# linto-ai/ssak

Hardware: AMD Instinct MI355X
Metric: utterances/sec (16 kHz, 10 s) Wav2Vec2-base CTC train step (higher is better)
Workload: dtype bf16; 1 GPU; Wav2Vec2-base CTC fine-tune step, bf16, synthetic 10 s @16 kHz utterances (BASELINE.json configs[1]; DP over xGMI for n_gpus>1 = configs[2]); per_gpu_batch=32, global_batch=32, samples_per_utt=160000, frames=499, frozen_feature_encoder=True, regularisers=script defaults (dropout/layerdrop/specaugment on), parallelism=dp1

## Files before the change

include/ssak_hip.h:

```cpp
#ifndef SSAK_HIP_H
#define SSAK_HIP_H
#include <stddef.h>
#include <stdint.h>

#ifdef __cplusplus
extern "C" {
#endif

#define SSAK_OK 0
#define SSAK_ERR_INVALID (-1)
#define SSAK_ERR_LAUNCH (-2)
#define SSAK_ERR_STATE (-3)

#define SSAK_REDUCTION_SUM 0
#define SSAK_REDUCTION_MEAN 1

int ssak_version(void);
const char* ssak_last_error(void);

size_t ssak_wave_normalize_workspace_bytes(int B, int T);
int ssak_wave_normalize(const float* in, const int32_t* lens, int B, int T, float* out, int32_t* mask,
                        void* workspace, size_t workspace_bytes, void* stream);

size_t ssak_logmel_table_floats(void);
// ... 344 lines not shown
int ssak_test_attn_adapter_fwd(const void* y, const void* res, const float* ln_g, const float* ln_b, const void* w1, const float* b1,
                               const void* w2, const float* b2, const float* next_g, const float* next_b, void* r_out, void* out,
                               float* mean, float* rstd, int M, int H, int A, float eps_adapter, float eps_next, int dtype,
                               void* stream);

int ssak_debug_posconv_prepare(const float* g, const float* v, void* wf, void* wb, float* norms, int H, int G, int K, int dtype,
                               void* stream);
int ssak_debug_posconv_pack(const void* h, void* pg, int B, int F, int H, int G, int K, int dtype, void* stream);
size_t ssak_debug_posconv_workspace_bytes(int B, int F, int H, int G, int K);
int ssak_debug_posconv_direct(const void* h, const void* w, const float* bias, void* out, void* pre, int B, int F, int H, int G, int K,
                              int row0, int gelu, void* workspace, size_t workspace_bytes, void* stream);
int ssak_debug_posconv_wgrad(const void* h, const void* dpre, float* dwf, int B, int F, int H, int G, int K, void* workspace,
                             size_t workspace_bytes, void* stream);
int ssak_debug_posconv_weight_bwd(const float* dwf, const float* g, const float* v, float* norms, float* dg, float* dv, int H, int G,
                                  int K, void* stream);

size_t ssak_debug_conv0_bwd_workspace_bytes(int B, int T, int C);
int ssak_debug_conv0_bwd(const float* x, const float* w, const float* gamma, const float* beta, const void* dy, const double* sums,
                         float* dw, float* dgamma, float* dbeta, int B, int T, int C, int dtype, void* workspace, size_t workspace_bytes,
                         void* stream);
size_t ssak_debug_conv0_wgrad_workspace_bytes(int B, int C, int ksize);
int ssak_debug_conv0_wgrad(const void* d, const float* x, float* dw, int B, int T, int C, int ksize, int stride, int dtype, void* workspace,
                           size_t workspace_bytes, void* stream);
int ssak_debug_conv0_bias(const float* x, const float* w, const float* bias, void* out, int B, int T, int C, int dtype, void* stream);
int ssak_debug_col2im(const void* dxcol, void* dx, int B, int Tin, int Tout, int C, int k, int s, int dtype, void* stream);
int ssak_debug_sum_slabs(const float* slabs, int nb, long n, float* out, void* stream);
int ssak_debug_conv_weight_rearrange(const float* w, void* out, int Co, int Ci, int k, int dtype, void* stream);
int ssak_debug_conv_wgrad_unrearrange(const float* dwr, float* g, int Co, int Ci, int k, void* stream);
int ssak_debug_col2im_k3s2(const void* dxcol, const void* pre, void* out, int B, int F, int Tin, int RS1, int H, int dtype, void* stream);
int ssak_debug_mel_to_cl(const float* mel, void* cl, int B, int C, int T, int RS, int lead, int dtype, void* stream);
// ... 8 lines not shown
```

ssak_amd/csrc/api.cpp:

```cpp
#include <stdarg.h>
#include <stdio.h>

#include <string.h>

#include <mutex>
#include <vector>

#include "kernels.h"

static thread_local char g_err[512] = "";

void ssak_set_error(const char* fmt, ...) {
  va_list ap;
  va_start(ap, fmt);
  vsnprintf(g_err, sizeof(g_err), fmt, ap);
  va_end(ap);
}

extern "C" int ssak_version(void) { return 630; }
extern "C" const char* ssak_last_error(void) { return g_err; }

#include <atomic>
#include <map>
namespace {
struct ProfRec {
  hipEvent_t e0, e1;
  int slot;
  double work;
};
struct ProfStream {
  int mode = 0;
  std::vector<char> want;
  std::vector<ProfRec> recs;
};
// ... 155 lines not shown
```

ssak_amd/csrc/kernels.h:

```cpp
#pragma once
#include "common.h"

enum : int {
  PROF_ATTN_FWD = 0, PROF_ATTN_BWD, PROF_LN_FWD, PROF_LN_BWD, PROF_CONV0, PROF_ADAMW, PROF_SUMSQ, PROF_CTC, PROF_WAVE_NORM,
  PROF_ROWWISE, PROF_POSCONV_W, PROF_SOFTMAX, PROF_POSCONV_DIRECT, PROF_POSCONV_WGRAD, PROF_LOGMEL,
  PROF_CLASS_SLOTS
};
constexpr int PROF_MAX_SLOTS = 128;
int ssak_prof_register(const char* name, int bound);
bool ssak_prof_wanted(int slot, hipStream_t st);
class ProfScope {
 public:
  ProfScope(int slot, double work, hipStream_t st);
  ~ProfScope();
  ProfScope(const ProfScope&) = delete;
  ProfScope& operator=(const ProfScope&) = delete;

 private:
  hipStream_t st_;
  hipEvent_t e0_ = nullptr;
  int slot_;
  double work_;
  bool on_;
};
// ... 49 lines not shown
                    hipStream_t st);
template <typename T>
int k_colsum_t(const T* X, long ld, int M, int N, float* out, hipStream_t st, float* scratch = nullptr, size_t scratch_floats = 0,
               const uint8_t* rowmask = nullptr, const int32_t* flens = nullptr, int F = 0);
int k_cast_f32_bf16(const float* in, bf16* out, long n, hipStream_t st);
template <typename T>
int k_specaug_fwd_t(T* h, const uint8_t* mask, const int32_t* flens, const float* embed, int B, int F, int C,
                    hipStream_t st);
template <typename T>
int k_specaug_bwd_t(T* dh, const uint8_t* mask, const int32_t* flens, float* dembed, int B, int F, int C,
                    hipStream_t st, float* scratch = nullptr, size_t scratch_floats = 0);
template <typename T>
int k_gelu_grad_mul_t(const T* dy, const T* pre, T* out, long n, hipStream_t st);
template <typename T>
int k_add_t(const T* a, const T* b, T* out, long n, hipStream_t st);
int k_layernorm_fwd(const bf16* y, const bf16* res, const float* gamma, const float* beta, bf16* r_out, bf16* out,
                    float* mean, float* rstd, int M, int C, float eps, const DropSpec& pre, const DropSpec& post,
                    hipStream_t st, const DropSpec& mid = DropSpec(), bool post_gelu = false);
int k_layernorm_bwd(const bf16* g1, const bf16* g2, const bf16* r, const float* mean, const float* rstd,
                    const float* gamma, const bf16* g_res, bf16* dr, bf16* dy, float* dgamma, float* dbeta,
                    float* partial, int M, int C, const DropSpec& pre, const DropSpec& post,
                    hipStream_t st, const DropSpec& mid = DropSpec(), float* dy_colsum = nullptr,
                    const float* post_gelu_beta = nullptr);
int k_colsum(const bf16* X, long ld, int M, int N, float* out, hipStream_t st, float* scratch = nullptr, size_t scratch_floats = 0,
             const uint8_t* rowmask = nullptr, const int32_t* flens = nullptr, int F = 0);

size_t k_conv0_stats_doubles(int B, int T0, int C);
template <typename T>
int k_conv0_gn_gelu_t(const float* x, const float* w, const float* gamma, const float* beta, T* out, double* stats,
                      int B, int Tn, int T0, int C, int ksize, int stride, hipStream_t st, bool raw_input = false);
// ... 77 lines not shown
```

ssak_amd/csrc/norm_act.hip:

```cpp
#include <algorithm>
#include <type_traits>

#include "common.h"
#include "kernels.h"

namespace {

SSAK_DEFINE_DROP_TABLE

constexpr int ROW_THREADS = 256;
template <int VEC>
__device__ __forceinline__ void load_colmul(uint32_t (&cm)[VEC], int col0) {
#pragma unroll
  for (int k = 0; k < VEC; k += 4) {
    const uint4 t = *reinterpret_cast<const uint4*>(g_drop_colmul.v + col0 + k);
    cm[k] = t.x, cm[k + 1] = t.y, cm[k + 2] = t.z, cm[k + 3] = t.w;
  }
}

template <typename T, int VEC>
using ChunkT = typename std::conditional<VEC == 8, Chunk8<T>, Chunk4<T>>::type;
template <typename T, int VEC>
__device__ __forceinline__ ChunkT<T, VEC> f_to_chunk(const float* f) {
  if constexpr (VEC == 8) return f_to_chunk8<T>(f);
// ... 604 lines not shown
}
__global__ __launch_bounds__(1024) void colsum_rows_kernel(const float* __restrict__ partial, int slots, int N, float* __restrict__ out) {
  __shared__ float red[16][65];
  const int cx = threadIdx.x & 63, ry = threadIdx.x >> 6;
  const int n = blockIdx.x * 64 + cx;
  float s = 0.f;
  if (n < N)
    for (int k = ry; k < slots; k += 16) s += partial[(long)k * N + n];
  red[ry][cx] = s;
  __syncthreads();
  if (ry == 0 && n < N) {
    float t = 0.f;
#pragma unroll
    for (int r = 0; r < 16; ++r) t += red[r][cx];
    out[n] += t;
  }
}

__global__ void cast_f32_bf16_kernel(const float* __restrict__ in, bf16* __restrict__ out, long n) {
  const long i = ((long)blockIdx.x * blockDim.x + threadIdx.x) * 4;
  if (i + 3 < n) {
    const float4 q = *reinterpret_cast<const float4*>(in + i);
    const bf16x4 t = {(bf16)q.x, (bf16)q.y, (bf16)q.z, (bf16)q.w};
    *reinterpret_cast<bf16x4*>(out + i) = t;
  } else {
    for (long j = i; j < n; ++j) out[j] = (bf16)in[j];
  }
}

template <typename T>
// ... 208 lines not shown
               const uint8_t* rowmask, const int32_t* flens, int F) {
  SSAK_REQUIRE(M > 0 && N > 0 && (N & 7) == 0 && (ld & 7) == 0, "colsum: N=%d ld=%ld must be multiples of 8", N, ld);
  dim3 grid(ssak_cdiv(N, 64), min(64, ssak_cdiv(M, 32)));
  ProfScope prof_scope(PROF_ROWWISE, (double)M * N * sizeof(T), st);
  const bool det = scratch && scratch_floats >= (size_t)grid.y * N;
  colsum_kernel<T><<<grid, 256, 0, st>>>(X, ld, M, N, out, det ? scratch : nullptr, rowmask, flens, F > 0 ? F : 1);
  SSAK_LAUNCH_CHECK();
  if (det) {
    if (g_reduce_sink && g_reduce_sink->push(scratch, N, (int)grid.y, N, out)) return SSAK_OK;
    colsum_rows_kernel<<<ssak_cdiv(N, 64), 1024, 0, st>>>(scratch, (int)grid.y, N, out);
    SSAK_LAUNCH_CHECK();
  }
  return SSAK_OK;
}

thread_local ReduceSink* g_reduce_sink = nullptr;

int k_colsum_rows(const float* partial, int slots, int N, float* out, hipStream_t st) {
  ProfScope prof_scope(PROF_ROWWISE, (double)slots * N * 4.0, st);
  colsum_rows_kernel<<<ssak_cdiv(N, 64), 1024, 0, st>>>(partial, slots, N, out);
  SSAK_LAUNCH_CHECK();
  return SSAK_OK;
}

int k_reduce_flush(ReduceSink& sink, hipStream_t st) {
  int done = 0;
  double bytes = 0.0;
  for (int i = 0; i < sink.n; ++i) bytes += (double)sink.jobs[i].slots * sink.jobs[i].ncols * 4.0;
  ProfScope prof_scope(PROF_ROWWISE, bytes, st);
  while (done < sink.n) {
// ... 64 lines not shown
  return SSAK_OK;
}

#define SSAK_INSTANTIATE_ROW_KERNELS(T)                                                                                           \
  template int k_layernorm_fwd_t<T>(const T*, const T*, const float*, const float*, T*, T*, float*, float*, int, int, float,      \
                                    const DropSpec&, const DropSpec&, hipStream_t, const DropSpec&, bool);                        \
  template int k_layernorm_bwd_t<T>(const T*, const T*, const T*, const float*, const float*, const float*, const T*, T*, T*,     \
                                    float*, float*, float*, int, int, const DropSpec&, const DropSpec&, hipStream_t,              \
                                    const DropSpec&, float*, const float*);                                                       \
  template int k_softmax_fwd_t<T>(const T*, T*, T*, const int32_t*, int, int, int, int, const DropSpec&, hipStream_t);            \
  template int k_softmax_bwd_t<T>(const T*, const T*, T*, int, int, int, const DropSpec&, hipStream_t);                           \
  template int k_colsum_t<T>(const T*, long, int, int, float*, hipStream_t, float*, size_t, const uint8_t*, const int32_t*, int); \
  template int k_specaug_fwd_t<T>(T*, const uint8_t*, const int32_t*, const float*, int, int, int, hipStream_t);                  \
  template int k_specaug_bwd_t<T>(T*, const uint8_t*, const int32_t*, float*, int, int, int, hipStream_t, float*, size_t);        \
  template int k_gelu_grad_mul_t<T>(const T*, const T*, T*, long, hipStream_t);                                                   \
  template int k_add_t<T>(const T*, const T*, T*, long, hipStream_t);
SSAK_INSTANTIATE_ROW_KERNELS(bf16)
SSAK_INSTANTIATE_ROW_KERNELS(float)

int k_layernorm_fwd(const bf16* y, const bf16* res, const float* gamma, const float* beta, bf16* r_out, bf16* out,
                    float* mean, float* rstd, int M, int C, float eps, const DropSpec& pre, const DropSpec& post,
                    hipStream_t st, const DropSpec& mid, bool post_gelu) {
  return k_layernorm_fwd_t<bf16>(y, res, gamma, beta, r_out, out, mean, rstd, M, C, eps, pre, post, st, mid, post_gelu);
}
int k_layernorm_bwd(const bf16* g1, const bf16* g2, const bf16* r, const float* mean, const float* rstd,
                    const float* gamma, const bf16* g_res, bf16* dr, bf16* dy, float* dgamma, float* dbeta,
                    float* partial, int M, int C, const DropSpec& pre, const DropSpec& post, hipStream_t st,
                    const DropSpec& mid, float* dy_colsum, const float* post_gelu_beta) {
  return k_layernorm_bwd_t<bf16>(g1, g2, r, mean, rstd, gamma, g_res, dr, dy, dgamma, dbeta, partial, M, C, pre, post, st, mid,
                                 dy_colsum, post_gelu_beta);
}
// ... 134 lines not shown
  SSAK_REQUIRE(debug_p_ok(p), "debug_softmax_bwd: p outside [0, 1)");
  const DropSpec d = debug_site(seed, site, p);
  if (dtype == 0) return k_softmax_bwd_t<bf16>((const bf16*)dPd, (const bf16*)P, (bf16*)dS, rows, cols, ld, d, (hipStream_t)stream);
  return k_softmax_bwd_t<float>((const float*)dPd, (const float*)P, (float*)dS, rows, cols, ld, d, (hipStream_t)stream);
}

extern "C" int ssak_debug_gelu(const float* x, long n, float* y, float* dydx, int dtype, void* stream) {
  SSAK_REQUIRE(dtype == 0 || dtype == 1, "debug_gelu: dtype %d (0 bf16, 1 fp32)", dtype);
  SSAK_REQUIRE(x && n > 0 && (y || dydx), "debug_gelu: bad arguments");
  const unsigned grid = (unsigned)((n + 255) / 256);
  if (dtype == 0) debug_gelu_kernel<bf16><<<grid, 256, 0, (hipStream_t)stream>>>(x, n, y, dydx);
  else debug_gelu_kernel<float><<<grid, 256, 0, (hipStream_t)stream>>>(x, n, y, dydx);
  SSAK_LAUNCH_CHECK();
  return SSAK_OK;
}
```

ssak_amd/csrc/optim.hip:

```cpp
#include "kernels.h"

namespace {

__global__ __launch_bounds__(256) void sumsq_kernel(const float* __restrict__ g, long n, float* __restrict__ out) {
  __shared__ float red[16];
  float s = 0.f;
  const long n4 = n >> 2;
  for (long i = (long)blockIdx.x * blockDim.x + threadIdx.x; i < n4; i += (long)gridDim.x * blockDim.x) {
    const float4 q = reinterpret_cast<const float4*>(g)[i];
    s += q.x * q.x + q.y * q.y + q.z * q.z + q.w * q.w;
  }
  if (blockIdx.x == 0)
    for (long i = (n4 << 2) + threadIdx.x; i < n; i += blockDim.x) s += g[i] * g[i];
  s = block_sum(s, red);
  if (threadIdx.x == 0) out[blockIdx.x] = s;
}
__global__ __launch_bounds__(1024) void sumsq_final_kernel(const float* __restrict__ partial, int n, float* __restrict__ out,
                                                           int add) {
  __shared__ float red[16];
  float s = threadIdx.x < n ? partial[threadIdx.x] : 0.f;
  s = block_sum(s, red);
  if (threadIdx.x == 0) out[0] = add ? out[0] + s : s;
}

__global__ __launch_bounds__(256) void adamw_kernel(float* __restrict__ p, const float* __restrict__ g,
                                                    float* __restrict__ m, float* __restrict__ v,
                                                    bf16* __restrict__ shadow, long n, const float* __restrict__ gnorm_sq,
                                                    float max_norm, float grad_scale, float lr, float beta1, float beta2,
                                                    float eps, float wd, float bc1, float bc2_sqrt) {
  float coef = grad_scale;
  if (gnorm_sq && max_norm > 0.f) {
    const float nrm = sqrtf(gnorm_sq[0]) * grad_scale;
    coef *= fminf(1.f, max_norm / (nrm + 1e-6f));
  }
  const float step_size = lr / bc1;
  const float decay = 1.f - lr * wd;
  const long n4 = n >> 2;
  for (long i = (long)blockIdx.x * blockDim.x + threadIdx.x; i < n4; i += (long)gridDim.x * blockDim.x) {
    float4 pp = reinterpret_cast<float4*>(p)[i];
    const float4 gg = reinterpret_cast<const float4*>(g)[i];
    float4 mm = reinterpret_cast<float4*>(m)[i];
    float4 vv = reinterpret_cast<float4*>(v)[i];
    float* pe = &pp.x;
    const float* ge = &gg.x;
    float* me = &mm.x;
    float* ve = &vv.x;
#pragma unroll
    for (int k = 0; k < 4; ++k) {
      const float gk = ge[k] * coef;
      me[k] = beta1 * me[k] + (1.f - beta1) * gk;
      ve[k] = beta2 * ve[k] + (1.f - beta2) * gk * gk;
      const float denom = sqrtf(ve[k]) / bc2_sqrt + eps;
      pe[k] = pe[k] * decay - step_size * (me[k] / denom);
    }
    reinterpret_cast<float4*>(p)[i] = pp;
    reinterpret_cast<float4*>(m)[i] = mm;
    reinterpret_cast<float4*>(v)[i] = vv;
    if (shadow) {
      const bf16x4 t = {(bf16)pp.x, (bf16)pp.y, (bf16)pp.z, (bf16)pp.w};
      reinterpret_cast<bf16x4*>(shadow)[i] = t;
    }
  }
  if (blockIdx.x == 0) {
    for (long i = (n4 << 2) + threadIdx.x; i < n; i += blockDim.x) {
      const float gk = g[i] * coef;
      const float mk = beta1 * m[i] + (1.f - beta1) * gk;
      const float vk = beta2 * v[i] + (1.f - beta2) * gk * gk;
      m[i] = mk;
      v[i] = vk;
      const float pk = p[i] * decay - step_size * (mk / (sqrtf(vk) / bc2_sqrt + eps));
      p[i] = pk;
      if (shadow) shadow[i] = (bf16)pk;
    }
  }
}

}

int k_sumsq(const float* g, long n, float* out, float* partial, hipStream_t st, bool add) {
  if (n <= 0) return SSAK_OK;
  const int blocks = (int)fmin(1024.0, (double)ssak_cdiv(n, 1024));
  ProfScope prof_scope(PROF_SUMSQ, (double)n * 4.0, st);
  sumsq_kernel<<<blocks, 256, 0, st>>>(g, n, partial);
  SSAK_LAUNCH_CHECK();
  sumsq_final_kernel<<<1, 1024, 0, st>>>(partial, blocks, out, add ? 1 : 0);
  SSAK_LAUNCH_CHECK();
  return SSAK_OK;
}

int k_adamw(float* p, const float* g, float* m, float* v, bf16* shadow, long n, const float* gnorm_sq, float max_norm,
            float grad_scale, float lr, float beta1, float beta2, float eps, float wd, int step, hipStream_t st) {
  if (n <= 0) return SSAK_OK;
  SSAK_REQUIRE(step >= 1, "adamw: step is 1-based");
  const float bc1 = 1.f - powf(beta1, (float)step);
  const float bc2s = sqrtf(1.f - powf(beta2, (float)step));
  ProfScope prof_scope(PROF_ADAMW, (double)n * (shadow ? 30.0 : 28.0), st);
  adamw_kernel<<<(int)fmin(4096.0, (double)ssak_cdiv(n, 1024)), 256, 0, st>>>(p, g, m, v, shadow, n, gnorm_sq, max_norm,
                                                                              grad_scale, lr, beta1, beta2, eps, wd, bc1, bc2s);
  SSAK_LAUNCH_CHECK();
  return SSAK_OK;
}

extern "C" int ssak_grad_sumsq(const float* grads, long n, float* out, void* workspace, size_t workspace_bytes, void* stream) {
  SSAK_REQUIRE(grads && out && n > 0, "grad_sumsq: bad arguments");
  SSAK_REQUIRE(((uintptr_t)grads & 15) == 0, "grad_sumsq: buffer must be 16-byte aligned");
  SSAK_REQUIRE(workspace && workspace_bytes >= 1024 * sizeof(float), "grad_sumsq: workspace of 4096 bytes needed");
  return k_sumsq(grads, n, out, (float*)workspace, (hipStream_t)stream);
}

extern "C" int ssak_grad_sumsq_add(const float* grads, long n, float* out, void* workspace, size_t workspace_bytes, void* stream) {
  SSAK_REQUIRE(grads && out && n > 0, "grad_sumsq_add: bad arguments");
  SSAK_REQUIRE(((uintptr_t)grads & 15) == 0, "grad_sumsq_add: buffer must be 16-byte aligned");
  SSAK_REQUIRE(workspace && workspace_bytes >= 1024 * sizeof(float), "grad_sumsq_add: workspace of 4096 bytes needed");
// ... 13 lines not shown
```

ssak_amd/csrc/w2v2_engine.hip:

```cpp
#include <algorithm>
#include <string>
#include <vector>
#include <string.h>

#include "kernels.h"

namespace {

constexpr int WGRAD_SETS = 3;

struct PInfo {
  std::string name;
  std::vector<long> shape;
  long offset = 0, numel = 0;
  int region = 0;
};

struct LayerP {
  long wqkv, bqkv, wo, bo, ln1w, ln1b, w1, b1, w2, b2, ln2w, ln2b;
  long ad_nw = 0, ad_nb = 0, ad_w1 = 0, ad_b1 = 0, ad_w2 = 0, ad_b2 = 0;
};

inline long align_up(long x, long a) { return (x + a - 1) / a * a; }

// ... 1185 lines not shown
  {
    const long span = (e->lp[0].w2 + (long)c.hidden_size * c.intermediate_size) - e->lp[0].wqkv;
    bool packed = true;
    for (int l = 1; l < c.num_layers; ++l) packed &= e->lp[l].wqkv == e->lp[l - 1].wqkv + span;
    const long w0 = e->lp[0].wqkv, w1 = e->lp[c.num_layers - 1].wqkv + span;
    if (!packed || w1 > n_grad) {
      SSAK_HIP(hipMemsetAsync(Gd, 0, (size_t)n_grad * sizeof(float), st));
    } else {
      if (w0 > 0) SSAK_HIP(hipMemsetAsync(Gd, 0, (size_t)w0 * sizeof(float), st));
      for (int l = 0; l < c.num_layers; ++l)
        if (!e->keep[l]) SSAK_HIP(hipMemsetAsync(Gd + e->lp[l].wqkv, 0, (size_t)span * sizeof(float), st));
      if (n_grad > w1) SSAK_HIP(hipMemsetAsync(Gd + w1, 0, (size_t)(n_grad - w1) * sizeof(float), st));
    }
  }
  AT* dlog = BF(p.dlog);
  if (dlogits) {
    if constexpr (EXACT)
      dlog = const_cast<float*>(dlogits);
    else
      TRY(k_cast_f32_bf16(dlogits, dlog, (long)M * V, st));
    TRY(k_colsum_t<AT>(dlog, V, M, V, Gd + e->p_lm_b, st, FP(p.lnpart), cs_floats));
  }
  auto announce = [&](long off, long cnt) {
    if (e->on_ready && cnt > 0) e->on_ready(off, cnt, e->on_ready_user);
  };
  const long layer_span = (e->lp[0].w2 + (long)H * I) - e->lp[0].wqkv;
  if (!dlogits) announce(e->p_lm_w, (long)V * H);
  AT* gA = BF(p.dA);
  AT* gB = nullptr;
  if (dhidden)
    SSAK_HIP(hipMemcpyAsync(gA, dhidden, (size_t)M * H * sizeof(AT), hipMemcpyDeviceToDevice, st));
  else {
    GemmX<EXACT> g(M, H, V);
    g.a(dlog, V).b(W + e->p_lm_w, H, true).c(gA, H);
    if (c.final_dropout > 0.f) g.drop(c.final_dropout, DS_FINAL, seed);
    TRY(g.run(st));
  }
  const bool stable = whisper || c.do_stable_layer_norm != 0;
  const AT* Gres = nullptr;
  auto free_buf = [&](const AT* u1, const AT* u2, const AT* u3) {
    AT* cand[3] = {BF(p.dC), BF(p.dA), BF(p.scratchH)};
    for (AT* cnd : cand)
      if (cnd != u1 && cnd != u2 && cnd != u3) return cnd;
    return (AT*)nullptr;
  };
  WgradQueue wq;
  ReduceSink sink;
// ... 186 lines not shown
    TRY(k_colsum_t<AT>(dpre2, H, M, H, Gd + e->p_c2b, st, FP(p.lnpart), cs_floats));
    TRY(k_copy_rows_padded_t<AT>(dpre2, BF(p.dpre2pad), B, F, RS2, H, st));
    TRY(GemmX<EXACT>(H, 3 * H, B * RS2).a(BF(p.dpre2pad), H, true).b(BF(p.h1pad), 2 * H, true).c(FP(p.dwr), 3 * H, true)
            .run_wgrad(st, slab, p.slab_bytes));
    TRY(k_conv_wgrad_unrearrange(FP(p.dwr), Gd + e->p_c2w, H, H, 3, st));
    TRY(GemmX<EXACT>(M, 3 * H, H).a(dpre2, H).b(e->conv_w[2], 3 * H, true).c(BF(p.dxcol), 3 * H).run(st));
    TRY(k_col2im_k3s2_t<AT>(BF(p.dxcol), BF(p.pre1), BF(p.dpre1pad), B, F, Tin, RS1, H, st));
    TRY(k_colsum_t<AT>(BF(p.dpre1pad), H, B * RS1, H, Gd + e->p_c1b, st, FP(p.lnpart), cs_floats));
    TRY(GemmX<EXACT>(H, 3 * NM, B * RS1).a(BF(p.dpre1pad), H, true).b(BF(p.melcl), NM, true).c(FP(p.dwr), 3 * NM, true)
            .run_wgrad(st, slab, p.slab_bytes));
    TRY(k_conv_wgrad_unrearrange(FP(p.dwr), Gd + e->p_c1w, H, NM, 3, st));
    for (int l = 0; l < c.num_layers; ++l)
      SSAK_HIP(hipMemsetAsync(Gd + e->lp[l].bqkv + H, 0, (size_t)H * sizeof(float), st));
   }
  } else {
  AT* dpre = BF(p.dY);
  TRY(k_gelu_grad_mul_t<AT>(dh1, BF(p.pc_pre), dpre, (long)M * H, st));
  TRY(k_colsum_t<AT>(dpre, H, M, H, Gd + e->p_pc_b, st, FP(p.lnpart), cs_floats));
  TRY(k_posconv_pack_t<AT>(dpre, BF(p.pgdy), B, F, H, G, K, st));
  {
    const int lead = K / 2, RS = F + K;
    bool pcw_direct = false;
    if constexpr (!EXACT)
      pcw_direct = e->posconv_direct && e->pc_wf_frag != nullptr && k_posconv_wgrad_scratch_floats(H, G, K) * sizeof(float) <= p.slab_bytes;
    if (pcw_direct) {
      if constexpr (!EXACT)
        TRY(k_posconv_wgrad_direct(BF(p.pgx), BF(p.pgdy), p.pg_rows, (long)B * RS, lead, FP(p.dwf), reinterpret_cast<float*>(slab), H, G, K, st));
    } else {
      TRY(GemmX<EXACT>(K * cg, cg, B * RS)
              .a(BF(p.pgx), cg, true)
              .b(BF(p.pgdy) + (long)lead * cg, cg, true)
              .c(FP(p.dwf), cg, true)
              .batch(1, G, 0, p.pg_rows * cg, 0, p.pg_rows * cg, 0, (long)cg * K * cg)
              .run(st));
// ... 88 lines not shown
```

ssak_amd/hip.py:

```python
from __future__ import annotations

import ctypes as C
import os

import numpy as np
import torch

_DEFAULT_LIB = os.path.join(os.path.dirname(os.path.abspath(__file__)), "lib", "libssak_hip.so")
_LIB_PATH = os.environ.get("SSAK_HIP_LIB") or _DEFAULT_LIB
ABI_VERSION = 630


class GemmDesc(C.Structure):
    _fields_ = [("M", C.c_int), ("N", C.c_int), ("K", C.c_int), ("a_kmajor", C.c_int), ("b_kmajor", C.c_int),
                ("lda", C.c_long), ("ldb", C.c_long), ("ldc", C.c_long), ("nb1", C.c_int), ("nb2", C.c_int),
                ("sa1", C.c_long), ("sa2", C.c_long), ("sb1", C.c_long), ("sb2", C.c_long), ("sc1", C.c_long),
                ("sc2", C.c_long), ("alpha", C.c_float), ("epilogue", C.c_int), ("out_f32", C.c_int),
                ("accumulate", C.c_int), ("split_k", C.c_int), ("drop_p", C.c_float), ("drop_stream", C.c_uint32),
                ("drop_seed", C.c_uint64), ("bias_s2", C.c_long), ("pads_are_zero", C.c_int), ("colsum", C.c_int),
                ("dynamic_tiles", C.c_int), ("b_fragments", C.c_void_p), ("plan_tile", C.c_int)]


class W2V2Config(C.Structure):
    _fields_ = [("vocab_size", C.c_int), ("hidden_size", C.c_int), ("num_layers", C.c_int), ("num_heads", C.c_int),
                ("intermediate_size", C.c_int), ("num_conv_layers", C.c_int), ("conv_dim", C.c_int * 8),
# ... 159 lines not shown
        "ssak_layernorm_fwd": (i32, [vp, vp, vp, vp, vp, vp, i32, i32, f32, i32, vp]),
        "ssak_debug_dropout_mask": (i32, [C.c_uint64, C.c_uint32, f32, C.c_long, i32, vp, C.POINTER(f32), vp]),
        "ssak_debug_attention_dropout_mask": (i32, [C.c_uint64, C.c_uint32, f32, i32, i32, i32, vp, vp]),
        "ssak_debug_layernorm_fwd": (i32, [vp, vp, vp, vp, vp, vp, vp, vp, i32, i32, f32, C.c_uint64, C.c_uint32, f32, C.c_uint32,
                                            f32, C.c_uint32, f32, i32, i32, vp]),
        "ssak_debug_layernorm_bwd_workspace_bytes": (sz, [i32]),
        "ssak_debug_layernorm_bwd": (i32, [vp, vp, vp, vp, vp, vp, vp, vp, vp, vp, vp, vp, vp, i32, i32, C.c_uint64, C.c_uint32, f32,
                                            C.c_uint32, f32, C.c_uint32, f32, i32, i32, vp, sz, vp]),
        "ssak_debug_softmax_fwd": (i32, [vp, vp, vp, vp, i32, i32, i32, i32, C.c_uint64, C.c_uint32, f32, i32, vp]),
        "ssak_debug_softmax_bwd": (i32, [vp, vp, vp, i32, i32, i32, C.c_uint64, C.c_uint32, f32, i32, vp]),
        "ssak_debug_gelu": (i32, [vp, C.c_long, vp, vp, i32, vp]),
        "ssak_test_attn_adapter_fwd": (i32, [vp, vp, vp, vp, vp, vp, vp, vp, vp, vp, vp, vp, vp, vp, i32, i32, i32, f32, f32, i32, vp]),
        "ssak_debug_posconv_prepare": (i32, [vp, vp, vp, vp, vp, i32, i32, i32, i32, vp]),
        "ssak_debug_posconv_pack": (i32, [vp, vp, i32, i32, i32, i32, i32, i32, vp]),
        "ssak_debug_posconv_workspace_bytes": (sz, [i32, i32, i32, i32, i32]),
        "ssak_debug_posconv_direct": (i32, [vp, vp, vp, vp, vp, i32, i32, i32, i32, i32, i32, i32, vp, sz, vp]),
        "ssak_debug_posconv_wgrad": (i32, [vp, vp, vp, i32, i32, i32, i32, i32, vp, sz, vp]),
        "ssak_debug_posconv_weight_bwd": (i32, [vp, vp, vp, vp, vp, vp, i32, i32, i32, vp]),
        "ssak_debug_conv0_bwd_workspace_bytes": (sz, [i32, i32, i32]),
        "ssak_debug_conv0_bwd": (i32, [vp, vp, vp, vp, vp, vp, vp, vp, vp, i32, i32, i32, i32, vp, sz, vp]),
        "ssak_debug_conv0_wgrad_workspace_bytes": (sz, [i32, i32, i32]),
        "ssak_debug_conv0_wgrad": (i32, [vp, vp, vp, i32, i32, i32, i32, i32, i32, vp, sz, vp]),
        "ssak_debug_conv0_bias": (i32, [vp, vp, vp, vp, i32, i32, i32, i32, vp]),
        "ssak_debug_col2im": (i32, [vp, vp, i32, i32, i32, i32, i32, i32, i32, vp]),
        "ssak_debug_sum_slabs": (i32, [vp, i32, C.c_long, vp, vp]),
        "ssak_debug_conv_weight_rearrange": (i32, [vp, vp, i32, i32, i32, i32, vp]),
        "ssak_debug_conv_wgrad_unrearrange": (i32, [vp, vp, i32, i32, i32, vp]),
        "ssak_debug_col2im_k3s2": (i32, [vp, vp, vp, i32, i32, i32, i32, i32, i32, vp]),
        "ssak_debug_mel_to_cl": (i32, [vp, vp, i32, i32, i32, i32, i32, i32, vp]),
        "ssak_debug_add_rowvec": (i32, [vp, vp, vp, i32, i32, i32, i32, vp]),
# ... 806 lines not shown
```

Baseline: 2229 utterances/sec.

## Fuse LM-head backward and posconv backward prologue; stream AdamW with nontemporal loads

Adds a fused LM-head backward kernel that casts the fp32 CTC logit gradient to bf16, computes the bias column sums, and runs the small-V input-gradient matmul with final dropout applied, all in one pass. A second fused kernel combines the GELU-gradient multiply, the column sum and the grouped-conv pack for the positional-conv backward, and zeroes the padding rows. AdamW is restructured to use contiguous per-block tiles, two-way unrolling and nontemporal loads and stores. The goal is to cut kernel launches and intermediate HBM round trips. The cost is custom MFMA code that carries its own correctness risk, and the LM-head kernel only runs in the bf16 path with V of 64 or less.

```diff
diff --git a/include/ssak_hip.h b/include/ssak_hip.h
--- a/include/ssak_hip.h
+++ b/include/ssak_hip.h
@@ -382,6 +382,11 @@
                              size_t workspace_bytes, void* stream);
 int ssak_debug_posconv_weight_bwd(const float* dwf, const float* g, const float* v, float* norms, float* dg, float* dv, int H, int G,
                                   int K, void* stream);
+int ssak_debug_lm_head_bwd(const float* dlogits, const void* W, void* dlog, void* gA, float* dbias, int M, int V, int H, uint64_t seed,
+                           uint32_t site, float p, void* workspace, size_t workspace_bytes, void* stream);
+size_t ssak_debug_posconv_bwd_prologue_workspace_bytes(int H);
+int ssak_debug_posconv_bwd_prologue(const void* dy, const void* pre, void* dpre, void* pgdy, float* dbias, int B, int F, int H, int G,
+                                    int K, int dtype, int fused, void* workspace, size_t workspace_bytes, void* stream);
 
 size_t ssak_debug_conv0_bwd_workspace_bytes(int B, int T, int C);
 int ssak_debug_conv0_bwd(const float* x, const float* w, const float* gamma, const float* beta, const void* dy, const double* sums,
diff --git a/ssak_amd/csrc/api.cpp b/ssak_amd/csrc/api.cpp
--- a/ssak_amd/csrc/api.cpp
+++ b/ssak_amd/csrc/api.cpp
@@ -17,7 +17,7 @@
   va_end(ap);
 }
 
-extern "C" int ssak_version(void) { return 630; }
+extern "C" int ssak_version(void) { return 640; }
 extern "C" const char* ssak_last_error(void) { return g_err; }
 
 #include <atomic>
diff --git a/ssak_amd/csrc/kernels.h b/ssak_amd/csrc/kernels.h
--- a/ssak_amd/csrc/kernels.h
+++ b/ssak_amd/csrc/kernels.h
@@ -87,6 +87,12 @@
 int k_gelu_grad_mul_t(const T* dy, const T* pre, T* out, long n, hipStream_t st);
 template <typename T>
 int k_add_t(const T* a, const T* b, T* out, long n, hipStream_t st);
+bool k_lm_head_bwd_supported(int V, int H);
+int k_lm_head_bwd(const float* dlogits, const bf16* W, bf16* dlog, bf16* gA, float* dbias, int M, int V, int H, const DropSpec& drop,
+                  hipStream_t st, float* scratch, size_t scratch_floats);
+template <typename T>
+int k_posconv_bwd_prologue_t(const T* dy, const T* pre, T* pgdy, float* dbias, int B, int F, int H, int G, int K, hipStream_t st,
+                             float* scratch, size_t scratch_floats);
 int k_layernorm_fwd(const bf16* y, const bf16* res, const float* gamma, const float* beta, bf16* r_out, bf16* out,
                     float* mean, float* rstd, int M, int C, float eps, const DropSpec& pre, const DropSpec& post,
                     hipStream_t st, const DropSpec& mid = DropSpec(), bool post_gelu = false);
diff --git a/ssak_amd/csrc/norm_act.hip b/ssak_amd/csrc/norm_act.hip
--- a/ssak_amd/csrc/norm_act.hip
+++ b/ssak_amd/csrc/norm_act.hip
@@ -642,6 +642,184 @@
 #pragma unroll
     for (int r = 0; r < 16; ++r) t += red[r][cx];
     out[n] += t;
+  }
+}
+
+template <typename T>
+__global__ __launch_bounds__(256) void posconv_bwd_prologue_kernel(const T* __restrict__ dy, const T* __restrict__ pre,
+                                                                   T* __restrict__ pg, float* __restrict__ partial, int B, int F,
+                                                                   int N, int cg, int K, int lead, int RS, long rows_total) {
+  __shared__ float red[32][65];
+  const int cx = threadIdx.x & 7, ry = threadIdx.x >> 3;
+  const int c0 = blockIdx.x * 64 + cx * 8;
+  const int M = B * F;
+  float acc[8] = {0.f, 0.f, 0.f, 0.f, 0.f, 0.f, 0.f, 0.f};
+  if (c0 < N) {
+    T* pgc = pg + (long)(c0 / cg) * rows_total * cg + c0 % cg;
+    for (int m = blockIdx.y * 32 + ry; m < M; m += gridDim.y * 32) {
+      float a[8], x[8], f[8];
+      chunk_to_f(ld8<T>(dy + (size_t)m * N + c0), a);
+      chunk_to_f(ld8<T>(pre + (size_t)m * N + c0), x);
+#pragma unroll
+      for (int k = 0; k < 8; ++k) a[k] *= gelu_grad_s<T>(x[k]);
+      const Chunk8<T> q = f_to_chunk8<T>(a);
+      st8<T>(pgc + (lead + (long)(m / F) * RS + m % F) * cg, q);
+      chunk_to_f(q, f);
+#pragma unroll
+      for (int k = 0; k < 8; ++k) acc[k] += f[k];
+    }
+  }
+#pragma unroll
+  for (int k = 0; k < 8; ++k) red[ry][cx * 8 + k] = acc[k];
+  __syncthreads();
+  if (threadIdx.x < 64) {
+    float s = 0.f;
+#pragma unroll
+    for (int r = 0; r < 32; ++r) s += red[r][threadIdx.x];
+    const int c = blockIdx.x * 64 + threadIdx.x;
+    if (c < N) partial[(size_t)blockIdx.y * N + c] = s;
+  }
+  const int cpr = N >> 3;
+  const long npad = ((long)lead + (long)(B + 1) * K) * cpr;
+  const Chunk8<T> zero = {};
+  for (long e = ((long)blockIdx.y * gridDim.x + blockIdx.x) * 256 + threadIdx.x; e < npad; e += (long)gridDim.x * gridDim.y * 256) {
+    const int c = (int)(e % cpr) * 8;
+    const long q = e / cpr;
+    long r = q;
+    if (q >= lead) {
+      const long b = (q - lead) / K, j = (q - lead) % K;
+      r = lead + b * RS + (b < B ? F : 0) + j;
+    }
+    st8<T>(pg + ((long)(c / cg) * rows_total + r) * cg + c % cg, zero);
+  }
+}
+
+constexpr int LMB_MAX_PAIRS = 6;
+constexpr int LMB_XP = 72;
+constexpr int LMB_GROUPS = 8;
+struct LmBwdParams {
+  const float* dlogits;
+  const bf16* W;
+  bf16* dlog;
+  bf16* gA;
+  float* partial;
+  int M, V, H, pairs;
+  uint64_t seed;
+  uint32_t stream, thresh;
+  float scale;
+};
+template <int KSTEPS>
+__global__ __launch_bounds__(1024) void lm_head_bwd_kernel(const LmBwdParams p) {
+  __shared__ __attribute__((aligned(16))) bf16 wfrag[LMB_MAX_PAIRS * 2 * 2 * 64 * 8];
+  __shared__ __attribute__((aligned(16))) bf16 xs[LMB_GROUPS * 32 * LMB_XP];
+  const int lane = threadIdx.x & 63, wave = threadIdx.x >> 6;
+  const int lc = lane & 15, g4 = lane >> 4;
+  const int by = blockIdx.x, ngy = gridDim.x;
+  const int h0 = blockIdx.y * p.pairs * 32;
+  for (int e = threadIdx.x; e < p.pairs * 2 * KSTEPS * 64; e += 1024) {
+    const int l = e & 63, ks = (e >> 6) % KSTEPS, u = ((e >> 6) / KSTEPS) & 1, q = (e >> 6) / KSTEPS / 2;
+    const int n = l & 15, h = h0 + 32 * q + 8 * (n >> 2) + 4 * u + (n & 3);
+    bf16x8 f;
+#pragma unroll
+    for (int i = 0; i < 8; ++i) {
+      const int k = 32 * ks + 8 * (l >> 4) + i;
+      f[i] = k < p.V ? p.W[(long)k * p.H + h] : (bf16)0.f;
+    }
+    *reinterpret_cast<bf16x8*>(wfrag + ((((long)q * 2 + u) * 2 + ks) * 64 + l) * 8) = f;
+  }
+  const int ngroups = (p.M + 31) >> 5;
+  const int mine = by < ngroups ? (ngroups - by + ngy - 1) / ngy : 0;
+  const int cr = threadIdx.x >> 5, cc = threadIdx.x & 31;
+  float cs0 = 0.f, cs1 = 0.f;
+  const uint32_t thi = p.thresh << 16;
+  const bool vec4 = (p.V & 3) == 0, vec8 = (p.V & 7) == 0;
+  for (int pass = 0; pass * LMB_GROUPS < mine; ++pass) {
+    const int gslot = wave >> 1, gi = pass * LMB_GROUPS + gslot;
+    const int m = (by + gi * ngy) * 32 + 16 * (wave & 1) + lc;
+    const bool live = gi < mine && m < p.M;
+    bf16x8 fd[KSTEPS];
+#pragma unroll
+    for (int ks = 0; ks < KSTEPS; ++ks) {
+      const int k0 = 32 * ks + 8 * g4;
+      const float* src = p.dlogits + (long)m * p.V + k0;
+      if (live && vec4 && k0 + 8 <= p.V) {
+        const f32x4 a = *reinterpret_cast<const f32x4*>(src), b = *reinterpret_cast<const f32x4*>(src + 4);
+        fd[ks] = (bf16x8){(bf16)a[0], (bf16)a[1], (bf16)a[2], (bf16)a[3], (bf16)b[0], (bf16)b[1], (bf16)b[2], (bf16)b[3]};
+      } else {
+#pragma unroll
+        for (int i = 0; i < 8; ++i) fd[ks][i] = (live && k0 + i < p.V) ? (bf16)src[i] : (bf16)0.f;
+      }
+    }
+    if (blockIdx.y == 0) {
+#pragma unroll
+      for (int ks = 0; ks < KSTEPS; ++ks) {
+        const int k0 = 32 * ks + 8 * g4;
+        bf16* dst = p.dlog + (long)m * p.V + k0;
+        if (live && vec8 && k0 + 8 <= p.V) {
+          *reinterpret_cast<bf16x8*>(dst) = fd[ks];
+        } else {
+#pragma unroll
+          for (int i = 0; i < 8; ++i)
+            if (live && k0 + i < p.V) dst[i] = fd[ks][i];
+        }
+        *reinterpret_cast<bf16x8*>(xs + (gslot * 32 + 16 * (wave & 1) + lc) * LMB_XP + k0) = fd[ks];
+      }
+    }
+    __syncthreads();
+    if (blockIdx.y == 0) {
+      for (int g = 0; g < LMB_GROUPS; ++g) {
+        const int gj = pass * LMB_GROUPS + g;
+        if (gj < mine && (by + gj * ngy) * 32 + cr < p.M) {
+          cs0 += (float)xs[(g * 32 + cr) * LMB_XP + cc];
+          if (KSTEPS > 1) cs1 += (float)xs[(g * 32 + cr) * LMB_XP + cc + 32];
+        }
+      }
+    }
+    if (gi < mine) {
+      const uint32_t rk = p.thresh ? drop_rowkey(p.seed, p.stream, (uint64_t)m) : 1u;
+      uint32_t cm[8], cmn[8];
+      if (p.thresh) load_colmul<8>(cmn, h0 + 8 * g4);
+      for (int q = 0; q < p.pairs; ++q) {
+        const int h = h0 + 32 * q + 8 * g4;
+        if (p.thresh) {
+#pragma unroll
+          for (int i = 0; i < 8; ++i) cm[i] = cmn[i];
+          if (q + 1 < p.pairs) load_colmul<8>(cmn, h + 32);
+        }
+        f32x4 acc[2];
+#pragma unroll
+        for (int u = 0; u < 2; ++u) {
+          acc[u] = (f32x4){0.f, 0.f, 0.f, 0.f};
+#pragma unroll
+          for (int ks = 0; ks < KSTEPS; ++ks) {
+            const bf16x8 fw = *reinterpret_cast<const bf16x8*>(wfrag + ((((long)q * 2 + u) * 2 + ks) * 64 + lane) * 8);
+            acc[u] = __builtin_amdgcn_mfma_f32_16x16x32_bf16(fw, fd[ks], acc[u], 0, 0, 0);
+          }
+        }
+        float v[8] = {acc[0][0], acc[0][1], acc[0][2], acc[0][3], acc[1][0], acc[1][1], acc[1][2], acc[1][3]};
+        if (p.thresh) {
+#pragma unroll
+          for (int i = 0; i < 8; ++i) v[i] = drop_keep(rk, cm[i], thi) ? v[i] * p.scale : 0.f;
+        }
+        bf16x8 o;
+#pragma unroll
+        for (int i = 0; i < 8; ++i) o[i] = (bf16)v[i];
+        if (live) *reinterpret_cast<bf16x8*>(p.gA + (long)m * p.H + h) = o;
+      }
+    }
+    __syncthreads();
+  }
+  if (blockIdx.y == 0) {
+    float* red = reinterpret_cast<float*>(xs);
+    red[cr * 64 + cc] = cs0;
+    red[cr * 64 + cc + 32] = cs1;
+    __syncthreads();
+    if (threadIdx.x < p.V) {
+      float s = 0.f;
+#pragma unroll
+      for (int r = 0; r < 32; ++r) s += red[r * 64 + threadIdx.x];
+      p.partial[(long)by * p.V + threadIdx.x] = s;
+    }
   }
 }
 
@@ -880,6 +1058,51 @@
   return SSAK_OK;
 }
 
+template <typename T>
+int k_posconv_bwd_prologue_t(const T* dy, const T* pre, T* pgdy, float* dbias, int B, int F, int H, int G, int K, hipStream_t st,
+                             float* scratch, size_t scratch_floats) {
+  SSAK_REQUIRE(B > 0 && F > 0 && G > 0 && K > 0 && H % G == 0 && (H / G) % 8 == 0,
+               "posconv_bwd_prologue: B=%d F=%d H=%d G=%d K=%d unsupported (H / G a multiple of 8)", B, F, H, G, K);
+  const int M = B * F, lead = K / 2, RS = F + K;
+  const long rows_total = lead + (long)B * RS + K;
+  dim3 grid(ssak_cdiv(H, 64), min(64, ssak_cdiv(M, 32)));
+  SSAK_REQUIRE(scratch && scratch_floats >= (size_t)grid.y * H, "posconv_bwd_prologue: scratch of %d floats needed", (int)grid.y * H);
+  ProfScope prof_scope(PROF_ROWWISE, (double)M * H * 3.0 * sizeof(T), st);
+  posconv_bwd_prologue_kernel<T><<<grid, 256, 0, st>>>(dy, pre, pgdy, scratch, B, F, H, H / G, K, lead, RS, rows_total);
+  SSAK_LAUNCH_CHECK();
+  if (g_reduce_sink && g_reduce_sink->push(scratch, H, (int)grid.y, H, dbias)) return SSAK_OK;
+  colsum_rows_kernel<<<ssak_cdiv(H, 64), 1024, 0, st>>>(scratch, (int)grid.y, H, dbias);
+  SSAK_LAUNCH_CHECK();
+  return SSAK_OK;
+}
+
+static int lm_head_bwd_slices(int H) {
+  const int total = H / 32;
+  for (int s = 1; s <= total; ++s)
+    if (total % s == 0 && total / s <= 6) return s;
+  return total;
+}
+bool k_lm_head_bwd_supported(int V, int H) { return V >= 1 && V <= 64 && H >= 32 && H % 32 == 0 && H <= DROP_TABLE_N; }
+
+int k_lm_head_bwd(const float* dlogits, const bf16* W, bf16* dlog, bf16* gA, float* dbias, int M, int V, int H, const DropSpec& drop,
+                  hipStream_t st, float* scratch, size_t scratch_floats) {
+  SSAK_REQUIRE(M > 0 && k_lm_head_bwd_supported(V, H), "lm_head_bwd: M=%d V=%d H=%d unsupported (V <= 64, H a multiple of 32)", M, V, H);
+  static_assert(6 <= LMB_MAX_PAIRS, "a slice's pairs fit wfrag");
+  const int ngy = min(64, ssak_cdiv(M, 32)), slices = lm_head_bwd_slices(H);
+  SSAK_REQUIRE(scratch && scratch_floats >= (size_t)ngy * V, "lm_head_bwd: scratch of %d floats needed", ngy * V);
+  LmBwdParams p{dlogits, W, dlog, gA, scratch, M, V, H, H / 32 / slices, drop.seed, drop.stream, thresh_of(drop.p), scale_of(drop.p)};
+  ProfScope prof_scope(PROF_ROWWISE, (double)M * (6.0 * V + 2.0 * H), st);
+  if (V <= 32)
+    lm_head_bwd_kernel<1><<<dim3(ngy, slices), 1024, 0, st>>>(p);
+  else
+    lm_head_bwd_kernel<2><<<dim3(ngy, slices), 1024, 0, st>>>(p);
+  SSAK_LAUNCH_CHECK();
+  if (g_reduce_sink && g_reduce_sink->push(scratch, V, ngy, V, dbias)) return SSAK_OK;
+  colsum_rows_kernel<<<ssak_cdiv(V, 64), 1024, 0, st>>>(scratch, ngy, V, dbias);
+  SSAK_LAUNCH_CHECK();
+  return SSAK_OK;
+}
+
 thread_local ReduceSink* g_reduce_sink = nullptr;
 
 int k_colsum_rows(const float* partial, int slots, int N, float* out, hipStream_t st) {
@@ -974,7 +1197,8 @@
   template int k_specaug_fwd_t<T>(T*, const uint8_t*, const int32_t*, const float*, int, int, int, hipStream_t);                  \
   template int k_specaug_bwd_t<T>(T*, const uint8_t*, const int32_t*, float*, int, int, int, hipStream_t, float*, size_t);        \
   template int k_gelu_grad_mul_t<T>(const T*, const T*, T*, long, hipStream_t);                                                   \
-  template int k_add_t<T>(const T*, const T*, T*, long, hipStream_t);
+  template int k_add_t<T>(const T*, const T*, T*, long, hipStream_t);                                                             \
+  template int k_posconv_bwd_prologue_t<T>(const T*, const T*, T*, float*, int, int, int, int, int, hipStream_t, float*, size_t);
 SSAK_INSTANTIATE_ROW_KERNELS(bf16)
 SSAK_INSTANTIATE_ROW_KERNELS(float)
 
@@ -1139,3 +1363,38 @@
   SSAK_LAUNCH_CHECK();
   return SSAK_OK;
 }
+
+extern "C" int ssak_debug_lm_head_bwd(const float* dlogits, const void* W, void* dlog, void* gA, float* dbias, int M, int V, int H,
+                                      uint64_t seed, uint32_t site, float p, void* workspace, size_t workspace_bytes, void* stream) {
+  SSAK_REQUIRE(dlogits && W && dlog && gA && dbias && workspace, "debug_lm_head_bwd: null pointer");
+  SSAK_REQUIRE(M > 0 && k_lm_head_bwd_supported(V, H) && (long)M * H < (1L << 31), "debug_lm_head_bwd: M=%d V=%d H=%d (V <= 64, H a multiple of 32)", M, V, H);
+  SSAK_REQUIRE(debug_p_ok(p), "debug_lm_head_bwd: p outside [0, 1)");
+  SSAK_REQUIRE(workspace_bytes >= (size_t)64 * V * sizeof(float), "debug_lm_head_bwd: workspace of 64 * V floats needed");
+  SSAK_HIP(hipMemsetAsync(dbias, 0, (size_t)V * sizeof(float), (hipStream_t)stream));
+  return k_lm_head_bwd(dlogits, (const bf16*)W, (bf16*)dlog, (bf16*)gA, dbias, M, V, H, debug_site(seed, site, p), (hipStream_t)stream,
+                       (float*)workspace, workspace_bytes / sizeof(float));
+}
+
+extern "C" size_t ssak_debug_posconv_bwd_prologue_workspace_bytes(int H) { return (size_t)64 * (H > 0 ? H : 0) * sizeof(float); }
+
+extern "C" int ssak_debug_posconv_bwd_prologue(const void* dy, const void* pre, void* dpre, void* pgdy, float* dbias, int B, int F, int H,
+                                               int G, int K, int dtype, int fused, void* workspace, size_t workspace_bytes,
+                                               void* stream) {
+  SSAK_REQUIRE(dtype == 0 || dtype == 1, "debug_posconv_bwd_prologue: dtype %d (0 bf16, 1 fp32)", dtype);
+  SSAK_REQUIRE(dy && pre && pgdy && dbias && workspace && (fused || dpre), "debug_posconv_bwd_prologue: null pointer");
+  SSAK_REQUIRE(B > 0 && F > 0 && G > 0 && K > 0 && H > 0 && H % G == 0 && (H / G) % 8 == 0 && (long)B * F * H < (1L << 31),
+               "debug_posconv_bwd_prologue: B=%d F=%d H=%d G=%d K=%d", B, F, H, G, K);
+  SSAK_REQUIRE(workspace_bytes >= ssak_debug_posconv_bwd_prologue_workspace_bytes(H), "debug_posconv_bwd_prologue: workspace too small");
+  hipStream_t st = (hipStream_t)stream;
+  float* ws = (float*)workspace;
+  const size_t wsf = workspace_bytes / sizeof(float);
+  SSAK_HIP(hipMemsetAsync(dbias, 0, (size_t)H * sizeof(float), st));
+  auto run = [&](auto* tag) -> int {
+    using T = std::remove_pointer_t<decltype(tag)>;
+    if (fused) return k_posconv_bwd_prologue_t<T>((const T*)dy, (const T*)pre, (T*)pgdy, dbias, B, F, H, G, K, st, ws, wsf);
+    if (int rc = k_gelu_grad_mul_t<T>((const T*)dy, (const T*)pre, (T*)dpre, (long)B * F * H, st)) return rc;
+    if (int rc = k_colsum_t<T>((const T*)dpre, H, B * F, H, dbias, st, ws, wsf)) return rc;
+    return k_posconv_pack_t<T>((const T*)dpre, (T*)pgdy, B, F, H, G, K, st);
+  };
+  return dtype == 0 ? run((bf16*)nullptr) : run((float*)nullptr);
+}
diff --git a/ssak_amd/csrc/optim.hip b/ssak_amd/csrc/optim.hip
--- a/ssak_amd/csrc/optim.hip
+++ b/ssak_amd/csrc/optim.hip
@@ -1,17 +1,40 @@
 #include "kernels.h"
 
 namespace {
+
+__device__ __forceinline__ f32x4 ld_stream(const float* p, long i4) {
+  return __builtin_nontemporal_load(reinterpret_cast<const f32x4*>(p) + i4);
+}
+__device__ __forceinline__ void st_stream(float* p, long i4, f32x4 v) {
+  __builtin_nontemporal_store(v, reinterpret_cast<f32x4*>(p) + i4);
+}
+
+__device__ __forceinline__ float rounded(float x) {
+  asm("" : "+v"(x));
+  return x;
+}
+__device__ __forceinline__ float sumsq4(f32x4 q) {
+  return rounded(q.x * q.x) + rounded(q.y * q.y) + rounded(q.z * q.z) + rounded(q.w * q.w);
+}
 
 __global__ __launch_bounds__(256) void sumsq_kernel(const float* __restrict__ g, long n, float* __restrict__ out) {
   __shared__ float red[16];
   float s = 0.f;
   const long n4 = n >> 2;
-  for (long i = (long)blockIdx.x * blockDim.x + threadIdx.x; i < n4; i += (long)gridDim.x * blockDim.x) {
-    const float4 q = reinterpret_cast<const float4*>(g)[i];
-    s += q.x * q.x + q.y * q.y + q.z * q.z + q.w * q.w;
+  const long step = (long)gridDim.x * blockDim.x;
+  long i = (long)blockIdx.x * blockDim.x + threadIdx.x;
+  for (; i + 3 * step < n4; i += 4 * step) {
+    f32x4 q[4];
+#pragma unroll
+    for (int u = 0; u < 4; ++u) q[u] = ld_stream(g, i + u * step);
+#pragma unroll
+    for (int u = 0; u < 4; ++u) s += sumsq4(q[u]);
+  }
+  for (; i < n4; i += step) {
+    s += sumsq4(ld_stream(g, i));
   }
   if (blockIdx.x == 0)
-    for (long i = (n4 << 2) + threadIdx.x; i < n; i += blockDim.x) s += g[i] * g[i];
+    for (long j = (n4 << 2) + threadIdx.x; j < n; j += blockDim.x) s = __builtin_fmaf(g[j], g[j], s);
   s = block_sum(s, red);
   if (threadIdx.x == 0) out[blockIdx.x] = s;
 }
@@ -23,52 +46,65 @@
   if (threadIdx.x == 0) out[0] = add ? out[0] + s : s;
 }
 
+struct AdamwScalars {
+  float coef, beta1, beta2, eps, bc2_sqrt, decay, step_size;
+};
+__device__ __forceinline__ void adamw_elem(const AdamwScalars& a, float& pk, float g, float& mk, float& vk) {
+  const float gk = g * a.coef;
+  mk = __builtin_fmaf(a.beta1, mk, (1.f - a.beta1) * gk);
+  vk = __builtin_fmaf(gk, (1.f - a.beta2) * gk, a.beta2 * vk);
+  const float denom = sqrtf(vk) / a.bc2_sqrt + a.eps;
+  pk = __builtin_fmaf(a.decay, pk, -(a.step_size * (mk / denom)));
+}
+
+constexpr int ADAMW_TILE = 256;
+
 __global__ __launch_bounds__(256) void adamw_kernel(float* __restrict__ p, const float* __restrict__ g,
                                                     float* __restrict__ m, float* __restrict__ v,
-                                                    bf16* __restrict__ shadow, long n, const float* __restrict__ gnorm_sq,
-                                                    float max_norm, float grad_scale, float lr, float beta1, float beta2,
-                                                    float eps, float wd, float bc1, float bc2_sqrt) {
+                                                    bf16* __restrict__ shadow, long n, long tiles_per_block,
+                                                    const float* __restrict__ gnorm_sq, float max_norm, float grad_scale,
+                                                    float lr, float beta1, float beta2, float eps, float wd, float bc1,
+                                                    float bc2_sqrt) {
   float coef = grad_scale;
-  if (gnorm_sq && max_norm > 0.f) {
-    const float nrm = sqrtf(gnorm_sq[0]) * grad_scale;
-    coef *= fminf(1.f, max_norm / (nrm + 1e-6f));
-  }
-  const float step_size = lr / bc1;
-  const float decay = 1.f - lr * wd;
+  if (gnorm_sq && max_norm > 0.f) coef *= fminf(1.f, max_norm / __builtin_fmaf(sqrtf(gnorm_sq[0]), grad_scale, 1e-6f));
+  AdamwScalars a;
+  a.coef = coef, a.beta1 = beta1, a.beta2 = beta2, a.eps = eps, a.bc2_sqrt = bc2_sqrt;
+  a.step_size = lr / bc1;
+  a.decay = __builtin_fmaf(-lr, wd, 1.f);
   const long n4 = n >> 2;
-  for (long i = (long)blockIdx.x * blockDim.x + threadIdx.x; i < n4; i += (long)gridDim.x * blockDim.x) {
-    float4 pp = reinterpret_cast<float4*>(p)[i];
-    const float4 gg = reinterpret_cast<const float4*>(g)[i];
-    float4 mm = reinterpret_cast<float4*>(m)[i];
-    float4 vv = reinterpret_cast<float4*>(v)[i];
-    float* pe = &pp.x;
-    const float* ge = &gg.x;
-    float* me = &mm.x;
-    float* ve = &vv.x;
+  const long first = (long)blockIdx.x * tiles_per_block * ADAMW_TILE;
+  const long last = first + tiles_per_block * ADAMW_TILE < n4 ? first + tiles_per_block * ADAMW_TILE : n4;
+  for (long i0 = first + threadIdx.x; i0 < last; i0 += 2 * ADAMW_TILE) {
+    const long i1 = i0 + ADAMW_TILE;
+    const bool two = i1 < last;
+    f32x4 pp[2], gg[2], mm[2], vv[2];
+    pp[0] = ld_stream(p, i0), gg[0] = ld_stream(g, i0), mm[0] = ld_stream(m, i0), vv[0] = ld_stream(v, i0);
+    if (two) pp[1] = ld_stream(p, i1), gg[1] = ld_stream(g, i1), mm[1] = ld_stream(m, i1), vv[1] = ld_stream(v, i1);
 #pragma unroll
-    for (int k = 0; k < 4; ++k) {
-      const float gk = ge[k] * coef;
-      me[k] = beta1 * me[k] + (1.f - beta1) * gk;
-      ve[k] = beta2 * ve[k] + (1.f - beta2) * gk * gk;
-      const float denom = sqrtf(ve[k]) / bc2_sqrt + eps;
-      pe[k] = pe[k] * decay - step_size * (me[k] / denom);
-    }
-    reinterpret_cast<float4*>(p)[i] = pp;
-    reinterpret_cast<float4*>(m)[i] = mm;
-    reinterpret_cast<float4*>(v)[i] = vv;
-    if (shadow) {
-      const bf16x4 t = {(bf16)pp.x, (bf16)pp.y, (bf16)pp.z, (bf16)pp.w};
-      reinterpret_cast<bf16x4*>(shadow)[i] = t;
+    for (int u = 0; u < 2; ++u) {
+      if (u == 1 && !two) break;
+      const long i = u ? i1 : i0;
+#pragma unroll
+      for (int k = 0; k < 4; ++k) {
+        float pk = pp[u][k], mk = mm[u][k], vk = vv[u][k];
+        adamw_elem(a, pk, gg[u][k], mk, vk);
+        pp[u][k] = pk, mm[u][k] = mk, vv[u][k] = vk;
+      }
+      st_stream(p, i, pp[u]);
+      st_stream(m, i, mm[u]);
+      st_stream(v, i, vv[u]);
+      if (shadow) {
+        const bf16x4 t = {(bf16)pp[u].x, (bf16)pp[u].y, (bf16)pp[u].z, (bf16)pp[u].w};
+        reinterpret_cast<bf16x4*>(shadow)[i] = t;
+      }
     }
   }
   if (blockIdx.x == 0) {
     for (long i = (n4 << 2) + threadIdx.x; i < n; i += blockDim.x) {
-      const float gk = g[i] * coef;
-      const float mk = beta1 * m[i] + (1.f - beta1) * gk;
-      const float vk = beta2 * v[i] + (1.f - beta2) * gk * gk;
+      float pk = p[i], mk = m[i], vk = v[i];
+      adamw_elem(a, pk, g[i], mk, vk);
       m[i] = mk;
       v[i] = vk;
-      const float pk = p[i] * decay - step_size * (mk / (sqrtf(vk) / bc2_sqrt + eps));
       p[i] = pk;
       if (shadow) shadow[i] = (bf16)pk;
     }
@@ -95,8 +131,11 @@
   const float bc1 = 1.f - powf(beta1, (float)step);
   const float bc2s = sqrtf(1.f - powf(beta2, (float)step));
   ProfScope prof_scope(PROF_ADAMW, (double)n * (shadow ? 30.0 : 28.0), st);
-  adamw_kernel<<<(int)fmin(4096.0, (double)ssak_cdiv(n, 1024)), 256, 0, st>>>(p, g, m, v, shadow, n, gnorm_sq, max_norm,
-                                                                              grad_scale, lr, beta1, beta2, eps, wd, bc1, bc2s);
+  const int tiles = ssak_cdiv(n, 1024);
+  const int tiles_per_block = ssak_cdiv(tiles, (int)fmin(4096.0, (double)ssak_cdiv(n, 1024)));
+  const int blocks = ssak_cdiv(tiles, tiles_per_block);
+  adamw_kernel<<<blocks, 256, 0, st>>>(p, g, m, v, shadow, n, tiles_per_block, gnorm_sq, max_norm, grad_scale, lr, beta1, beta2,
+                                       eps, wd, bc1, bc2s);
   SSAK_LAUNCH_CHECK();
   return SSAK_OK;
 }
diff --git a/ssak_amd/csrc/w2v2_engine.hip b/ssak_amd/csrc/w2v2_engine.hip
--- a/ssak_amd/csrc/w2v2_engine.hip
+++ b/ssak_amd/csrc/w2v2_engine.hip
@@ -1223,12 +1223,19 @@
     }
   }
   AT* dlog = BF(p.dlog);
+  bool lm_fused = false;
   if (dlogits) {
-    if constexpr (EXACT)
+    if constexpr (EXACT) {
       dlog = const_cast<float*>(dlogits);
-    else
-      TRY(k_cast_f32_bf16(dlogits, dlog, (long)M * V, st));
-    TRY(k_colsum_t<AT>(dlog, V, M, V, Gd + e->p_lm_b, st, FP(p.lnpart), cs_floats));
+    } else {
+      lm_fused = k_lm_head_bwd_supported(V, H);
+      if (lm_fused)
+        TRY(k_lm_head_bwd(dlogits, W + e->p_lm_w, dlog, BF(p.dA), Gd + e->p_lm_b, M, V, H,
+                          c.final_dropout > 0.f ? DS(c.final_dropout, DS_FINAL) : none, st, FP(p.lnpart), cs_floats));
+      else
+        TRY(k_cast_f32_bf16(dlogits, dlog, (long)M * V, st));
+    }
+    if (!lm_fused) TRY(k_colsum_t<AT>(dlog, V, M, V, Gd + e->p_lm_b, st, FP(p.lnpart), cs_floats));
   }
   auto announce = [&](long off, long cnt) {
     if (e->on_ready && cnt > 0) e->on_ready(off, cnt, e->on_ready_user);
@@ -1239,7 +1246,7 @@
   AT* gB = nullptr;
   if (dhidden)
     SSAK_HIP(hipMemcpyAsync(gA, dhidden, (size_t)M * H * sizeof(AT), hipMemcpyDeviceToDevice, st));
-  else {
+  else if (!lm_fused) {
     GemmX<EXACT> g(M, H, V);
     g.a(dlog, V).b(W + e->p_lm_w, H, true).c(gA, H);
     if (c.final_dropout > 0.f) g.drop(c.final_dropout, DS_FINAL, seed);
@@ -1456,10 +1463,7 @@
       SSAK_HIP(hipMemsetAsync(Gd + e->lp[l].bqkv + H, 0, (size_t)H * sizeof(float), st));
    }
   } else {
-  AT* dpre = BF(p.dY);
-  TRY(k_gelu_grad_mul_t<AT>(dh1, BF(p.pc_pre), dpre, (long)M * H, st));
-  TRY(k_colsum_t<AT>(dpre, H, M, H, Gd + e->p_pc_b, st, FP(p.lnpart), cs_floats));
-  TRY(k_posconv_pack_t<AT>(dpre, BF(p.pgdy), B, F, H, G, K, st));
+  TRY(k_posconv_bwd_prologue_t<AT>(dh1, BF(p.pc_pre), BF(p.pgdy), Gd + e->p_pc_b, B, F, H, G, K, st, FP(p.lnpart), cs_floats));
   {
     const int lead = K / 2, RS = F + K;
     bool pcw_direct = false;
diff --git a/ssak_amd/hip.py b/ssak_amd/hip.py
--- a/ssak_amd/hip.py
+++ b/ssak_amd/hip.py
@@ -8,7 +8,7 @@
 
 _DEFAULT_LIB = os.path.join(os.path.dirname(os.path.abspath(__file__)), "lib", "libssak_hip.so")
 _LIB_PATH = os.environ.get("SSAK_HIP_LIB") or _DEFAULT_LIB
-ABI_VERSION = 630
+ABI_VERSION = 640
 
 
 class GemmDesc(C.Structure):
@@ -198,6 +198,9 @@
         "ssak_debug_posconv_prepare": (i32, [vp, vp, vp, vp, vp, i32, i32, i32, i32, vp]),
         "ssak_debug_posconv_pack": (i32, [vp, vp, i32, i32, i32, i32, i32, i32, vp]),
         "ssak_debug_posconv_workspace_bytes": (sz, [i32, i32, i32, i32, i32]),
+        "ssak_debug_lm_head_bwd": (i32, [vp, vp, vp, vp, vp, i32, i32, i32, C.c_uint64, C.c_uint32, f32, vp, sz, vp]),
+        "ssak_debug_posconv_bwd_prologue_workspace_bytes": (sz, [i32]),
+        "ssak_debug_posconv_bwd_prologue": (i32, [vp, vp, vp, vp, vp, i32, i32, i32, i32, i32, i32, i32, vp, sz, vp]),
         "ssak_debug_posconv_direct": (i32, [vp, vp, vp, vp, vp, i32, i32, i32, i32, i32, i32, i32, vp, sz, vp]),
         "ssak_debug_posconv_wgrad": (i32, [vp, vp, vp, i32, i32, i32, i32, i32, vp, sz, vp]),
         "ssak_debug_posconv_weight_bwd": (i32, [vp, vp, vp, vp, vp, vp, i32, i32, i32, vp]),
```

After: 2248 utterances/sec, median of 6. About the same (+0.9%).
